# gicheonkang/gst-visdial

Hardware: AMD Instinct MI355X
Metric: dialog-rounds/sec (enc_dec_a train step) (higher is better)
Workload: dtype bf16; 1 GPU; enc_dec_a train step (fwd+loss+bwd+allreduce+AdamW, dropout on), 16 rows/GPU, seq_len 256, 37x2048 region features, answer len 25 [BASELINE configs[1] per-GPU shape]; global_batch=16, rows_per_gpu=16, seq_len=256, parallelism=dp1, hip_graph=True, optimizer_update=in the weight-gradient launch's epilogue + remainder pass, payload_written_by_wgrad_launch=False, capture_quiesce=no-process-group, full=False

## Files before the change

### gst_visdial_amd/_lib.py

```python
import ctypes as C
import os

_HERE = os.path.dirname(os.path.abspath(__file__))
LIB_PATH = os.path.join(_HERE, "lib", "libgstvd_hip.so")
ABI_VERSION = 9

F32, BF16 = 0, 1
EPI_BIAS, EPI_ADD, EPI_GELU, EPI_DGELU, EPI_DROPOUT = 1, 2, 4, 8, 16
EPI_COLSUM, EPI_COLSUM_ACC = 32, 64
EPI_ADAMW = 128
LN_RESID, LN_EMBED, LN_IMAGE = 0, 1, 2

_vp, _i64, _i32, _f32, _u32 = C.c_void_p, C.c_int64, C.c_int32, C.c_float, C.c_uint32


class GemmDesc(C.Structure):
    _fields_ = [("A", _vp), ("B", _vp), ("C", _vp), ("bias", _vp), ("addend", _vp), ("aux", _vp),
                ("M", _i64), ("N", _i64), ("K", _i64),
                ("lda", _i64), ("ldb", _i64), ("ldc", _i64), ("ldadd", _i64), ("ldaux", _i64),
                ("batch", _i64), ("sA", _i64), ("sB", _i64), ("sC", _i64), ("sAdd", _i64), ("sAux", _i64),
                ("dtype_in", _i32), ("dtype_out", _i32), ("a_kmajor", _i32), ("b_kmajor", _i32), ("epilogue", _i32),
                ("alpha", _f32), ("dropout_p", _f32), ("site", _u32), ("rng", _vp)]


# ... 76 lines not shown
    _fields_ = [("partial", _vp), ("out", _vp * 3), ("nblk", _i64), ("stride", _i64), ("H", _i64),
                ("nvec", _i32), ("accumulate", _i32 * 3), ("blk0", _i32)]


class SlabEntry(C.Structure):
    _fields_ = [("x", _vp), ("scratch", _vp), ("ldx", _i64), ("M", _i64), ("N", _i64), ("blk0", _i32), ("pad_", _i32)]


SIGNATURES = {
    "gstvd_abi_version": (_i32, []),
    "gstvd_build_arch": (C.c_char_p, []),
    "gstvd_gemm": (_i32, [C.POINTER(GemmDesc), _vp]),
    "gstvd_gemm_splitk_ws_bytes": (_i64, [_i64, _i64, _i32]),
    "gstvd_gemm_splitk": (_i32, [_vp, _i32, _vp, _i64, _vp]),
    "gstvd_gemm_group_tile": (_i32, []),
    "gstvd_gemm_group_caps": (_i32, []),
    "gstvd_gemv_ln": (_i32, [C.POINTER(GemmDesc), _vp, _vp, _f32, _vp, _i64, _vp]),
    "gstvd_gemm_kernel_name": (_i32, [C.POINTER(GemmDesc), _i32, C.c_char_p, _i32]),
    "gstvd_gemm_grouped_kernel_name": (_i32, [_i32, _i32, _i32, _i32, C.c_char_p, _i32]),
    "gstvd_gemm_grouped": (_i32, [_vp, _vp, _i64, _i64, _i32, _i32, _i32, _i32, _vp, _i64, _vp]),
    "gstvd_ln_fwd": (_i32, [C.POINTER(LnDesc), _vp]),
    "gstvd_ln_bwd_blocks": (_i64, [_i64]),
    "gstvd_ln_bwd_blocks_for": (_i64, [_i64, _i64, _i32]),
    "gstvd_ln_bwd": (_i32, [C.POINTER(LnBwdDesc), _vp]),
    "gstvd_gemm_ln_fwd": (_i32, [C.POINTER(GemmDesc), C.POINTER(LnDesc), _vp]),
    "gstvd_gemm_ln_bwd": (_i32, [C.POINTER(GemmDesc), C.POINTER(LnBwdDesc), _vp]),
    "gstvd_gemm_ln_rows_per_block": (_i64, []),
    "gstvd_colsum_partials": (_i32, [_vp, _i64, _i64, _i64, _vp, _vp, _vp, _i32, _vp]),
    "gstvd_colsum_batched": (_i32, [_vp, _i64, _i64, _vp]),
    "gstvd_colsum_slabs_batched": (_i32, [_vp, _i64, _i64, _i32, _vp]),
    "gstvd_colsum_slabs": (_i32, [_vp, _i64, _i64, _i64, _i32, _vp, _i64, _vp]),
    "gstvd_colsum": (_i32, [_vp, _i64, _i64, _i64, _i32, _vp, _vp, _i64, _i32, _vp]),
    "gstvd_locgrad": (_i32, [_vp, _i64, _vp, _i64, _i64, _i32, _vp, _i32, _vp]),
    "gstvd_attn_fwd": (_i32, [C.POINTER(AttnDesc), _vp]),
    "gstvd_attn_bwd": (_i32, [C.POINTER(AttnDesc), _vp]),
    "gstvd_ln_kernel_name": (_i32, [_vp, _i32, C.c_char_p, _i32]),
    "gstvd_attn_kernel_name": (_i32, [C.POINTER(AttnDesc), _i32, C.c_char_p, _i32]),
    "gstvd_ce_fwd": (_i32, [_vp, _i64, _vp, _i64, _i64, _i64, _i32, _vp, _vp, _vp, _vp]),
    "gstvd_ce_bwd": (_i32, [_vp, _i64, _vp, _vp, _vp, _vp, _i32, _i64, _i64, _i64, _i32, _vp, _i64, _vp]),
    "gstvd_ce_bwd_rows": (_i32, [_vp, _i64, _vp, _vp, _vp, _i64, _i64, _i64, _i32, _vp, _i64, _vp]),
    "gstvd_fgsm_step": (_i32, [_vp, _vp, _f32, _vp, _i64, _vp]),
    "gstvd_answer_scores": (_i32, [_vp, _i64, _vp, _vp, _i64, _i64, _i32, _vp, _vp]),
    "gstvd_sample_topk": (_i32, [C.POINTER(SampleDesc), _vp]),
    "gstvd_vl_split": (_i32, [_vp, _i64, _i64, _i64, _i64, _i32, _vp, _vp, _f32, _u32, _u32, _vp, _vp]),
    "gstvd_cast": (_i32, [_vp, _i32, _vp, _i32, _i64, _vp]),
    "gstvd_cast_ranges": (_i32, [_vp, _vp, _vp, _vp, _i64, _i64, _vp]),
    "gstvd_scale": (_i32, [_vp, _vp, _i64, _vp]),
    "gstvd_rng_advance": (_i32, [_vp, _vp]),
    "gstvd_dropout_mask": (_i32, [_vp, _i64, _f32, _u32, _vp, _vp]),
    "gstvd_adamw": (_i32, [_vp, _vp, _vp, _vp, _vp, _i64, _vp, _vp, _i64, _f32, _f32, _f32, _vp, _f32, _i64, _vp]),
    "gstvd_adamw_bf16grad": (_i32, [_vp, _vp, _i64, _vp, _vp, _vp, _i64, _vp, _vp, _i64, _f32, _f32, _f32, _vp, _f32, _i64, _vp]),
    "gstvd_adamw_blocks": (_i32, [_vp, _vp, _vp, _vp, _vp, _i64, _vp, _vp, _i64, _f32, _f32, _f32, _vp, _f32, _i64, _vp, _i64, _vp, _vp]),
    "gstvd_gemm_grouped_adamw": (_i32, [_vp, _vp, _i64, _i64, C.POINTER(AdamFuse), _vp, _i64, _vp]),
    "gstvd_gemm_grouped_adamw_kernel_name": (_i32, [C.c_char_p, _i32]),
    "gstvd_nsp_head": (_i32, [C.POINTER(NspHeadDesc), _vp]),
    "gstvd_rows_gather": (_i32, [_vp, _i64, _i64, _vp, _i64, _i64, _i32, _vp, _i64, _vp]),
    "gstvd_rows_scatter": (_i32, [_vp, _i64, _vp, _i64, _i64, _i32, _vp, _i64, _i64, _i32, _vp]),
    "gstvd_rows_mul": (_i32, [_vp, _i64, _vp, _i64, _i64, _i64, _i32, _vp]),
    "gstvd_kl_fwd": (_i32, [_vp, _i64, _vp, _i64, _vp, _vp, _i64, _i64, _i32, _vp, _vp, _vp, _vp]),
    "gstvd_kl_bwd": (_i32, [_vp, _i64, _vp, _i64, _vp, _vp, _vp, _vp, _vp, _i32, _i64, _i64, _i32, _vp, _i64, _vp]),
    "gstvd_nsp_train_fwd": (_i32, [C.POINTER(NspTrainDesc), _vp]),
    "gstvd_nsp_train_bwd": (_i32, [C.POINTER(NspTrainDesc), _vp]),
    "gstvd_beam_step": (_i32, [C.POINTER(BeamStepDesc), _vp]),
    "gstvd_beam_reorder": (_i32, [C.POINTER(BeamReorderDesc), _vp]),
}

_STATUS = {-1: "GSTVD_E_DTYPE", -2: "GSTVD_E_SHAPE", -3: "GSTVD_E_ALIGN", -4: "GSTVD_E_NULL", -5: "GSTVD_E_UNSUPPORTED"}


class GstvdError(RuntimeError):
    pass


_lib = None


def load():
    global _lib
    if _lib is not None:
        return _lib
    if not os.path.exists(LIB_PATH):
        raise GstvdError(
            "gst_visdial_amd: HIP library %s not found; build it first (make -C gst_visdial_amd/csrc). "
            "There is no CPU fallback for the product path." % LIB_PATH)
    import torch
    lib = C.CDLL(LIB_PATH)
    for name, (res, args) in SIGNATURES.items():
        fn = getattr(lib, name)
        fn.restype = res
        fn.argtypes = args
    if lib.gstvd_abi_version() != ABI_VERSION:
        raise GstvdError("libgstvd_hip.so ABI %d != expected %d; rebuild" % (lib.gstvd_abi_version(), ABI_VERSION))
    _lib = lib
    return lib


N_CALLS = [0]


def check(name, rc):
    N_CALLS[0] += 1
    if rc != 0:
        what = _STATUS.get(rc, "hipError_t %d" % rc if rc > 0 else "status %d" % rc)
        raise GstvdError("%s failed: %s" % (name, what))
```

### gst_visdial_amd/csrc/gemm_dma256.hip

```cpp
#include "gemm_common.h"

static __device__ __attribute__((aligned(256))) char g_zero_page256[256];
static constexpr int g_strip_w = 8;
constexpr int NS256 = 3;

DEVFN int opaque_lane(int lane) { asm volatile("" : "+v"(lane)); return lane; }
DEVFN int rm32_off(int row, int slot) { return row * 64 + ((slot ^ (((row >> 3) & 1) << 1)) << 4); }
template <int BX> DEVFN int km32_off(int krow, int col) {
  constexpr int NB = BX / 16;
  const int f = (krow & 3) | (((krow >> 3) & 1) << 2);
  return krow * (BX * 2) + ((((col >> 4) ^ f) & (NB - 1)) << 5) + ((col & 15) << 1);
}

template <int BX, bool KM> DEVFN bf16x8 frag32(const char* img, int xb, int lane) {
  const int g = lane >> 4, li = lane & 15;
  if (!KM) {
    return *(const bf16x8*)(img + rm32_off(xb + li, g));
  } else {
    const int kr = 8 * g + (li >> 2), col = xb + 4 * (lane & 3);
    s16x4 lo = lds_tr16(img + km32_off<BX>(kr, col));
    s16x4 hi = lds_tr16(img + km32_off<BX>(kr + 4, col));
    typedef __attribute__((ext_vector_type(8))) short s16x8;
    s16x8 v = {lo[0], lo[1], lo[2], lo[3], hi[0], hi[1], hi[2], hi[3]};
    return __builtin_bit_cast(bf16x8, v);
// ... 106 lines not shown
  }
#pragma unroll
  for (int i = 0; i < MI; ++i)
#pragma unroll
    for (int j = 0; j < NI; ++j)
      gemm_epilogue_tile<bf16, OT>(p, dk, acc[i][j], z, m0 + wm * WTM + i * 16 + li, n0 + wn * WTN + j * 16 + 4 * g);
}

#ifndef ADAMW_PARK_DEPTH
#define ADAMW_PARK_DEPTH 5
#endif
template <int NI, int ROWS, int D>
DEVFN void adamw_rows_pass(const gstvd_adamw_fuse_t& af, float alpha, float lr, float wd, float bc, const float* park, int64_t flat0,
                           int rows_left, int cols_left, unsigned ldc, int lane) {
  static_assert(NI == 4, "16 lanes x 4 columns = the wave tile's 64 columns");
  constexpr int S = epi_row_floats<NI>(), RPI = 4, R = ROWS / RPI;
  if (rows_left <= 0 || cols_left <= 0) return;
  const int rl = lane >> 4, c4 = (lane & 15) * 4;
  const bool n_ok = c4 < cols_left;
  float* Pt = af.param + flat0; float* Mt = af.m + flat0; float* Vt = af.v + flat0;
  bf16* St = (bf16*)af.shadow_bf16 + flat0;
  float* Gt = const_cast<float*>(af.grad_base) + flat0;
  const unsigned cofs = n_ok ? (unsigned)c4 : 0u;
  const int last = rows_left - 1;
  f32x4 bm[D + 1], bv[D + 1], bp[D + 1];
  auto fetch = [&](int rr, int b) {
    const int row = rr * RPI + rl;
    const unsigned o = (unsigned)(row < last ? row : last) * ldc + cofs;
    bm[b] = __builtin_nontemporal_load((const f32x4*)(Mt + o)); bv[b] = __builtin_nontemporal_load((const f32x4*)(Vt + o));
    bp[b] = __builtin_nontemporal_load((const f32x4*)(Pt + o));
  };
#pragma unroll
  for (int k = 0; k < D; ++k) fetch(k, k);
#pragma unroll
  for (int rr = 0; rr < R; ++rr) {
    if (rr + D < R) fetch(rr + D, (rr + D) % (D + 1));
    const int b = rr % (D + 1);
    const int row = rr * RPI + rl;
    f32x4 g4 = *(const f32x4*)(park + row * S + c4);
    g4 = g4 * alpha;
    f32x4 p4 = bp[b], m4 = bm[b], v4 = bv[b];
    adamw_update4(p4, m4, v4, g4, af.grad_scale, lr, wd, bc, af.beta1, af.beta2, af.eps);
    if (row < rows_left && n_ok) {
      const unsigned o = (unsigned)row * ldc + (unsigned)c4;
      if (af.write_grad) st4(Gt + o, g4);
      __builtin_nontemporal_store(m4, (f32x4*)(Mt + o));
      __builtin_nontemporal_store(v4, (f32x4*)(Vt + o));
      __builtin_nontemporal_store(p4, (f32x4*)(Pt + o));
      if (af.shadow_bf16) st4(St + o, p4);
    }
  }
}

template <typename OT, bool AKM, bool BKM, int NIU = 4, bool CS = false, bool ADAM = false>
DEVFN void pc_tile256(const GemmP& p, int64_t z, int wg, int ntn, int nwg, char* smem, const gstvd_adamw_fuse_t af = gstvd_adamw_fuse_t{}) {
  constexpr int BM = 256, BN = 256, WN = 4, NS = NS256, NTP = 256;
  constexpr int WTM = 128, WTN = NIU * 16, MI = 8, NI = NIU, BNU = WN * WTN;
  constexpr int A_BYTES = BM * 64, B_BYTES = BN * 64, STAGE = A_BYTES + B_BYTES;
  constexpr int NPA = A_BYTES / (NTP * 16), NPB = B_BYTES / (NTP * 16), LPS = NPA + NPB;
  static_assert((NS - 2) * LPS <= 63, "vmcnt immediate out of range");

  const int tid = threadIdx.x, lane = tid & 63;
  const int wave = __builtin_amdgcn_readfirstlane(tid >> 6);
  const bool producer = wave >= 8;
  const int ntm = nwg / ntn;
  const int SWD = g_strip_w;
  const int strip = wg / (SWD * ntm), sw = (ntn - strip * SWD) < SWD ? (ntn - strip * SWD) : SWD;
  const int within = wg - strip * SWD * ntm;
  const int64_t m0 = (int64_t)(within / sw) * BM, n0 = (int64_t)(strip * SWD + within % sw) * BNU;
  const int64_t nkt = (p.K + 31) / 32;

  if (producer) {
    const int ptid = tid - 512, pw = wave - 8;
    Dma32<BM, AKM, NPA, NTP> ua;
    Dma32<BN, BKM, NPB, NTP> ub;
    ua.init(p.A + z * p.sA * 2, p.lda, m0, p.M, ptid);
    ub.init(p.B + z * p.sB * 2, p.ldb, n0, (n0 + BNU < p.N) ? n0 + BNU : p.N, ptid);
#pragma unroll
    for (int s = 0; s < NS - 1; ++s) {
      ua.issue(s, p.K, smem + s * STAGE, pw);
      ub.issue(s, p.K, smem + s * STAGE + A_BYTES, pw);
    }
    int fill = NS - 1, slot = 0;
    const bool do_cs = CS && AKM && (p.epi & GSTVD_EPI_COLSUM) && n0 == 0 && p.bias != nullptr;
    const int rg = lane >> 3, cg = pw * 8 + (lane & 7);
    float cs[8] = {0.f, 0.f, 0.f, 0.f, 0.f, 0.f, 0.f, 0.f};
    for (int64_t t = 0; t < nkt; ++t) {
      asm volatile("s_waitcnt vmcnt(%0)" ::"n"((NS - 2) * LPS) : "memory");
      __builtin_amdgcn_s_barrier();
      asm volatile("" ::: "memory");
      ua.issue(t + NS - 1, p.K, smem + fill * STAGE, pw);
      ub.issue(t + NS - 1, p.K, smem + fill * STAGE + A_BYTES, pw);
      if (CS && do_cs) {
        const char* cA = smem + slot * STAGE;
#pragma unroll
        for (int r = 0; r < 4; ++r) {
          const bf16x8 v = *(const bf16x8*)(cA + km32_off<BM>(rg * 4 + r, cg * 8));
#pragma unroll
          for (int e = 0; e < 8; ++e) cs[e] += (float)v[e];
        }
        asm volatile("s_waitcnt lgkmcnt(0)" ::: "memory");
      }
      fill = (fill + 1 == NS) ? 0 : fill + 1;
      slot = (slot + 1 == NS) ? 0 : slot + 1;
    }
    asm volatile("s_waitcnt vmcnt(0)" ::: "memory");
    __builtin_amdgcn_s_barrier();
    if (CS && do_cs) {
#pragma unroll
      for (int e = 0; e < 8; ++e) {
        float v = cs[e];
        v += __shfl_xor(v, 8, 64);
        v += __shfl_xor(v, 16, 64);
        v += __shfl_xor(v, 32, 64);
        cs[e] = v;
      }
      if (rg == 0) {
// ... 213 lines not shown
          const bf16x8 fa = *(const bf16x8*)(cA + rm64_off(wm * WTM + i * 16 + li, h * 4 + g));
#pragma unroll
          for (int j = 0; j < NI; ++j) acc[i][j] = mfma_bf16_k32(fb[j], fa, acc[i][j]);
        }
      }
    }
    sa = (sa + 1 == 3) ? 0 : sa + 1;
    sb ^= 1;
  }
  }
  __builtin_amdgcn_s_barrier();
  const int lane_e = sizeof(OT) == 4 ? opaque_lane(lane) : lane;
  const int g = lane_e >> 4, li = lane_e & 15;
  const DropKey dk = make_drop((p.epi & GSTVD_EPI_DROPOUT) ? p.p : 0.f, p.site, p.rng);
  if constexpr (sizeof(OT) == 2) {
    if (epilogue_rows_ok(p)) {
      gemm_epilogue_rows<MI, NI, 4, (NIU >= 4)>(p, dk, acc, z, m0 + wm * WTM, n0 + wn * WTN, smem + wave * epi_wave_bytes<NI, 4>(), lane_e);
      return;
    }
  }
#pragma unroll
  for (int i = 0; i < MI; ++i) {
    const int li_i = opaque_lane(li), g_i = opaque_lane(g);
#pragma unroll
    for (int j = 0; j < NI; ++j)
      gemm_epilogue_tile<bf16, OT>(p, dk, acc[i][j], z, m0 + wm * WTM + i * 16 + li_i, n0 + wn * WTN + j * 16 + 4 * g_i);
  }
}

DEVFN int xcd_remap256(int bid, int nwg) {
  const int xcd = bid & 7, q = nwg >> 3, r = nwg & 7;
  return (xcd < r ? xcd * (q + 1) : r * (q + 1) + (xcd - r) * q) + (bid >> 3);
}

template <typename OT, bool AKM, bool BKM, int NIU = 4>
__global__ __launch_bounds__(512) void gemm_dma256_kernel(GemmP p, int ntn, int nwg) {
  extern __shared__ __attribute__((aligned(16))) char smem[];
  dma_tile256<OT, AKM, BKM, NIU>(p, blockIdx.y, xcd_remap256(blockIdx.x, nwg), ntn, nwg, smem);
}

template <typename OT, bool AKM, bool BKM, int NIU = 4>
__global__ __launch_bounds__(768) void gemm_pc256_kernel(GemmP p, int ntn, int nwg) {
  extern __shared__ __attribute__((aligned(16))) char smem[];
  pc_tile256<OT, AKM, BKM, NIU>(p, blockIdx.y, xcd_remap256(blockIdx.x, nwg), ntn, nwg, smem);
}

template <typename OT, int NIU>
__global__ __launch_bounds__(768) void gemm_pc256_nt64_kernel(GemmP p, int ntn, int nwg) {
  extern __shared__ __attribute__((aligned(16))) char smem[];
  pc_tile256_nt64<OT, NIU>(p, blockIdx.y, xcd_remap256(blockIdx.x, nwg), ntn, nwg, smem);
}

constexpr int GROUP_TILE_MASK = 0x1fffff;
DEVFN int grouped_tile_id(const int* bmap, int total, int chs) {
  const int bid = blockIdx.x;
  if (bmap) return bmap[bid];
  const int full = total - total % (8 << chs);
  return bid < full ? (((bid >> 3) >> chs) * 8 + (bid & 7)) * (1 << chs) + ((bid >> 3) & ((1 << chs) - 1)) : bid;
}

DEVFN GemmP grouped_problem(const gstvd_gemm_t* tab, const int* tile_off, int nprob, int gid, int& tile, int& ntn, int& nwg) {
  int lo = 0, hi = nprob - 1;
  while (lo < hi) { const int mid = (lo + hi + 1) >> 1; if (tile_off[mid] <= gid) lo = mid; else hi = mid - 1; }
  const gstvd_gemm_t& g = tab[lo];
  GemmP p;
  p.A = (const char*)g.A; p.B = (const char*)g.B; p.C = (char*)g.C;
  p.bias = g.bias; p.addend = (const char*)g.addend; p.aux = (char*)g.aux;
  p.M = g.M; p.N = g.N; p.K = g.K;
  p.lda = g.lda; p.ldb = g.ldb; p.ldc = g.ldc; p.ldadd = g.ldadd; p.ldaux = g.ldaux;
  p.sA = p.sB = p.sC = p.sAdd = p.sAux = 0;
  p.epi = g.epilogue; p.alpha = g.alpha; p.p = g.dropout_p; p.site = g.site; p.rng = g.rng;
  ntn = (int)((g.N + 255) / 256);
  nwg = (int)((g.M + 255) / 256) * ntn;
  tile = gid - tile_off[lo];
  return p;
}

template <typename OT, bool AKM, bool BKM>
__global__ __launch_bounds__(768) void gemm_pc256_grouped_kernel(const gstvd_gemm_t* tab, const int* tile_off, int nprob, int total, int chs,
                                                                 const int* bmap) {
  extern __shared__ __attribute__((aligned(16))) char smem[];
  const int entry = grouped_tile_id(bmap, total, chs);
  if (entry < 0 || (entry & GROUP_TILE_MASK) >= total) return;
  int tile, ntn, nwg;
  const GemmP p = grouped_problem(tab, tile_off, nprob, entry & GROUP_TILE_MASK, tile, ntn, nwg);
  pc_tile256<OT, AKM, BKM, 4, true>(p, 0, tile, ntn, nwg, smem);
}

__global__ __launch_bounds__(768) void gemm_pc256_grouped_adamw_kernel(const gstvd_gemm_t* tab, const int* tile_off, int nprob, int total, int chs,
                                                                       const int* bmap, gstvd_adamw_fuse_t af) {
  extern __shared__ __attribute__((aligned(16))) char smem[];
  const int entry = grouped_tile_id(bmap, total, chs);
  if (entry < 0 || (entry & GROUP_TILE_MASK) >= total) return;
  int tile, ntn, nwg;
  const GemmP p = grouped_problem(tab, tile_off, nprob, entry & GROUP_TILE_MASK, tile, ntn, nwg);
  pc_tile256<float, true, true, 4, true, true>(p, 0, tile, ntn, nwg, smem, af);
}

constexpr int RING256 = NS256 * (256 + 256) * 64;
constexpr int PARK256 = 8 * epi_wave_bytes<4, 4>();
constexpr int LDS256 = RING256 > PARK256 ? RING256 : PARK256;
constexpr int64_t PC256_MAX_TILES = 512;
constexpr int64_t GEMM256_MIN_TILES = 120;
constexpr int GROUP_CHUNK_LOG2 = 3;

template <typename OT, bool AKM, bool BKM>
static int launch256(const GemmP& p, int64_t batch, int niu, hipStream_t s) {
  const int bnu = niu == 3 ? 192 : 256;
  const int ntm = (int)((p.M + 255) / 256), ntn = (int)((p.N + bnu - 1) / bnu);
  const dim3 grid((unsigned)(ntm * ntn), (unsigned)batch);
  if ((int64_t)ntm * ntn * batch > PC256_MAX_TILES) {
    auto k4 = gemm_dma256_kernel<OT, AKM, BKM, 4>;
    auto k3 = gemm_dma256_kernel<OT, AKM, BKM, 3>;
    static int attr_rc = ensure_lds(k4, LDS256) | ensure_lds(k3, LDS256);
    if (attr_rc) return attr_rc;
    GSTVD_LAUNCH(bnu == 192 ? k3 : k4, grid, dim3(512), LDS256, s, p, ntn, ntm * ntn);
    GSTVD_LAUNCH_CHECK();
    return 0;
  }
  if constexpr (!AKM && !BKM) {
    if (p.K % 64 == 0 && p.K >= 128) {
      auto n4 = gemm_pc256_nt64_kernel<OT, 4>;
      auto n3 = gemm_pc256_nt64_kernel<OT, 3>;
      constexpr int L4 = 3 * 256 * 128 + 2 * 256 * 128, L3 = 3 * 256 * 128 + 2 * 192 * 128;
      constexpr int P4 = 8 * epi_wave_bytes<4, 4>(), P3 = 8 * epi_wave_bytes<3, 4>();
      constexpr int lds4 = L4 > P4 ? L4 : P4, lds3 = L3 > P3 ? L3 : P3;
      static_assert(lds4 <= 160 * 1024 && lds3 <= 160 * 1024, "LDS budget");
      static int nt_rc = ensure_lds(n4, lds4) | ensure_lds(n3, lds3);
      if (nt_rc) return nt_rc;
      GSTVD_LAUNCH(bnu == 192 ? n3 : n4, grid, dim3(768), bnu == 192 ? lds3 : lds4, s, p, ntn, ntm * ntn);
      GSTVD_LAUNCH_CHECK();
      return 0;
    }
  }
  auto c4 = gemm_pc256_kernel<OT, AKM, BKM, 4>;
  auto c3 = gemm_pc256_kernel<OT, AKM, BKM, 3>;
  static int pc_rc = ensure_lds(c4, LDS256) | ensure_lds(c3, LDS256);
  if (pc_rc) return pc_rc;
  GSTVD_LAUNCH(bnu == 192 ? c3 : c4, grid, dim3(768), LDS256, s, p, ntn, ntm * ntn);
  GSTVD_LAUNCH_CHECK();
  return 0;
}

template <typename OT>
static int launch256_layout(const GemmP& p, int64_t batch, int akm, int bkm, int niu, hipStream_t s) {
  if (!akm && !bkm) return launch256<OT, false, false>(p, batch, niu, s);
  if (!akm && bkm) return launch256<OT, false, true>(p, batch, niu, s);
  if (akm && bkm) return launch256<OT, true, true>(p, batch, niu, s);
  return GSTVD_E_UNSUPPORTED;
}

static int pick_niu(const GemmP& p, int64_t batch) {
  const double nkt = (double)((p.K + 31) / 32), ntm = (double)((p.M + 255) / 256);
  const double t4 = ntm * (double)((p.N + 255) / 256) * batch, t3 = ntm * (double)((p.N + 191) / 192) * batch;
  const double r4 = (double)(int64_t)((t4 + 255) / 256), r3 = (double)(int64_t)((t3 + 255) / 256);
  return r3 * (14.0 + 0.84 * nkt) < r4 * (14.0 + 0.95 * nkt) ? 3 : 4;
}

int gemm_dma256_dispatch(const GemmP& p, int64_t batch, int akm, int bkm, int out_f32, hipStream_t s) {
  const int64_t tiles = ((p.M + 255) / 256) * ((p.N + 255) / 256) * batch;
  if (p.M < 256 || p.N < 256 || tiles < GEMM256_MIN_TILES) return GSTVD_E_UNSUPPORTED;
  const int niu = pick_niu(p, batch);
  return out_f32 ? launch256_layout<float>(p, batch, akm, bkm, niu, s) : launch256_layout<bf16>(p, batch, akm, bkm, niu, s);
}

template <typename OT, bool AKM, bool BKM>
static int grouped256(const gstvd_gemm_t* tab, const int* off, int nprob, int total, const int* bmap, int nblocks, hipStream_t s) {
  auto kp = gemm_pc256_grouped_kernel<OT, AKM, BKM>;
  static int pc_rc = ensure_lds(kp, LDS256);
  if (pc_rc) return pc_rc;
  GSTVD_LAUNCH(kp, dim3((unsigned)(bmap ? nblocks : total)), dim3(768), LDS256, s, tab, off, nprob, total, GROUP_CHUNK_LOG2, bmap);
  GSTVD_LAUNCH_CHECK();
  return 0;
}

extern "C" int gstvd_gemm_group_tile(void) { return 256; }

extern "C" int32_t gstvd_gemm_group_caps(void) { return 1; }

extern "C" int gstvd_gemm_grouped_kernel_name(int32_t dtype_in, int32_t dtype_out, int32_t a_kmajor, int32_t b_kmajor, char* buf,
                                              int32_t buf_len) {
  if (!buf || buf_len <= 1) return GSTVD_E_NULL;
  const void* fn = nullptr;
  static gstvd_gemm_t dummy_tab;
  static int32_t dummy_off;
  gstvd_plan_capture = &fn;
  const int rc = gstvd_gemm_grouped(&dummy_tab, &dummy_off, 1, 1, dtype_in, dtype_out, a_kmajor, b_kmajor, nullptr, 0, nullptr);
  gstvd_plan_capture = nullptr;
  if (rc) return rc;
  return copy_kernel_name(fn, buf, buf_len);
}

extern "C" int gstvd_gemm_grouped_adamw_kernel_name(char* buf, int32_t buf_len) {
  if (!buf || buf_len <= 1) return GSTVD_E_NULL;
  return copy_kernel_name((const void*)gemm_pc256_grouped_adamw_kernel, buf, buf_len);
}

extern "C" int gstvd_gemm_grouped_adamw(const gstvd_gemm_t* table_dev, const int32_t* tile_off_dev, int64_t nprob, int64_t total_tiles,
                                        const gstvd_adamw_fuse_t* f, const int32_t* block_map_dev, int64_t nblocks, gstvd_stream_t stream) {
  if (!table_dev || !tile_off_dev || !f) return GSTVD_E_NULL;
  if (!f->grad_base || !f->param || !f->m || !f->v || !f->step) return GSTVD_E_NULL;
  if (nprob <= 0 || total_tiles <= 0) return GSTVD_E_SHAPE;
  if (block_map_dev && (nblocks < total_tiles || total_tiles > GROUP_TILE_MASK)) return GSTVD_E_SHAPE;
  if (((uintptr_t)f->grad_base | (uintptr_t)f->param | (uintptr_t)f->m | (uintptr_t)f->v | (uintptr_t)f->shadow_bf16) & 15) return GSTVD_E_ALIGN;
  auto kp = gemm_pc256_grouped_adamw_kernel;
  static int rc = ensure_lds(kp, LDS256);
  if (rc) return rc;
  GSTVD_LAUNCH(kp, dim3((unsigned)(block_map_dev ? nblocks : total_tiles)), dim3(768), LDS256, (hipStream_t)stream, table_dev, tile_off_dev,
               (int)nprob, (int)total_tiles, GROUP_CHUNK_LOG2, block_map_dev, *f);
  GSTVD_LAUNCH_CHECK();
  return 0;
}

extern "C" int gstvd_gemm_grouped(const gstvd_gemm_t* table_dev, const int32_t* tile_off_dev, int64_t nprob, int64_t total_tiles,
                                  int32_t dtype_in, int32_t dtype_out, int32_t a_kmajor, int32_t b_kmajor,
                                  const int32_t* block_map_dev, int64_t nblocks, gstvd_stream_t stream) {
  if (!table_dev || !tile_off_dev) return GSTVD_E_NULL;
  if (nprob <= 0 || total_tiles <= 0) return GSTVD_E_SHAPE;
  if (block_map_dev && (nblocks < total_tiles || total_tiles > GROUP_TILE_MASK)) return GSTVD_E_SHAPE;
  if (dtype_in != GSTVD_BF16) return GSTVD_E_UNSUPPORTED;
  hipStream_t s = (hipStream_t)stream;
  const int n = (int)nprob, t = (int)total_tiles, nb = (int)nblocks;
  const int* bm = block_map_dev;
  if (dtype_out == GSTVD_F32) {
    if (a_kmajor && b_kmajor) return grouped256<float, true, true>(table_dev, tile_off_dev, n, t, bm, nb, s);
    if (!a_kmajor && b_kmajor) return grouped256<float, false, true>(table_dev, tile_off_dev, n, t, bm, nb, s);
    if (!a_kmajor && !b_kmajor) return grouped256<float, false, false>(table_dev, tile_off_dev, n, t, bm, nb, s);
  } else if (dtype_out == GSTVD_BF16) {
    if (a_kmajor && b_kmajor) return grouped256<bf16, true, true>(table_dev, tile_off_dev, n, t, bm, nb, s);
    if (!a_kmajor && b_kmajor) return grouped256<bf16, false, true>(table_dev, tile_off_dev, n, t, bm, nb, s);
    if (!a_kmajor && !b_kmajor) return grouped256<bf16, false, false>(table_dev, tile_off_dev, n, t, bm, nb, s);
  }
  return GSTVD_E_UNSUPPORTED;
}
```

### gst_visdial_amd/ops.py

```python
import ctypes as C

import torch

from . import _lib as L
from ._lib import F32, BF16, EPI_BIAS, EPI_ADD, EPI_GELU, EPI_DGELU, EPI_DROPOUT, LN_RESID, LN_EMBED, LN_IMAGE

_DT = {torch.float32: F32, torch.bfloat16: BF16}


def dt(t):
    return _DT[t.dtype]


def _p(t):
    if t is None:
        return None
    if not t.is_cuda:
        raise L.GstvdError("gst_visdial_amd ops need GPU tensors (got %s); there is no CPU path" % t.device)
    return t.data_ptr()


_RAW_STREAM = getattr(torch._C, "_cuda_getCurrentRawStream", None)
_DEV_INDEX = None

# ... 261 lines not shown

    def add(self, A, B, C_out, M, N, K, accumulate, colsum_out=None, colsum_acc=False):
        di, do = dt(A), dt(C_out)
        if self.items and (di, do) != (self.dtype_in, self.dtype_out):
            self.flush()
        self.dtype_in, self.dtype_out = di, do
        self.keep.append((A, B, C_out, colsum_out))
        cs = (_p(colsum_out), int(bool(colsum_acc))) if colsum_out is not None else (0, 0)
        self.items.append((_p(A), _p(B), _p(C_out), M, N, K, A.stride(-2), B.stride(-2), C_out.stride(-2), int(bool(accumulate))) + cs)

    def reset(self):
        self.items, self.keep = [], []

    def pending_into(self, C_out):
        ptr = _p(C_out)
        return any(it[2] == ptr for it in self.items)

    @staticmethod
    def _overlapping(items):
        spans = sorted((it[2], it[2] + 4 * ((it[3] - 1) * it[8] + it[4]), i) for i, it in enumerate(items))
        bad, reach, owner = set(), -1, -1
        for lo, hi, i in spans:
            if lo < reach:
                bad.add(i); bad.add(owner)
            if hi > reach:
                reach, owner = hi, i
        return bad

    def flush_direct_bf16(self, G, Gb):
        if not self.items or self.dtype_in != BF16 or self.dtype_out != F32 or not (self.a_km and self.b_km):
            self.flush()
            return ()
        base, nG = G.data_ptr(), G.numel()
        shared = self._overlapping(self.items)
        direct, rest, keep_d, keep_r, ranges = [], [], [], [], []
        for i, (it, kp) in enumerate(zip(self.items, self.keep)):
            (a, b, c, M, N, K, lda, ldb, ldc, acc) = it[:10]
            off = (c - base) // 4
            if acc or i in shared or ldc != N or c < base or off + M * N > nG or (c - base) % 4 or off % 8:
                rest.append(it); keep_r.append(kp)
            else:
                direct.append(it[:2] + (Gb.data_ptr() + 2 * off,) + it[3:]); keep_d.append(kp)
                ranges.append((off, M * N))
        self.items, self.keep = rest, keep_r
        self.flush()
        if direct:
            self.items, self.keep, self.dtype_out = direct, keep_d, BF16
            try:
                self.flush()
            finally:
                self.dtype_out = F32
        return tuple(sorted(ranges))

    def flush(self, fuse=None):
        if not self.items:
            return ()
        keep, self.keep = self.keep, []
        fused = ()
        if fuse is not None and self.dtype_in == BF16 and self.dtype_out == F32 and self.a_km and self.b_km:
            items, fl = [], []
            shared = self._overlapping(self.items)
            for i, it in enumerate(self.items):
                (a, b, c, M, N, K, lda, ldb, ldc, acc, cs_ptr, cs_acc) = it[:12]
                hp_addr, offs = (0, ()) if (acc or i in shared) else fuse.cover(c, M, N, ldc)
                fl.extend(offs)
                items.append(it[:12] + (hp_addr,))
            if fl:
                self.items, fused = items, tuple(fl)
            else:
                fuse = None
        else:
            fuse = None
        if self.dtype_in != BF16:
            lib = L.load()
            for (a, b, c, M, N, K, lda, ldb, ldc, acc, cs_ptr, cs_acc) in [it[:12] for it in self.items]:
                if cs_ptr:
                    raise L.GstvdError("column sums ride on the grouped bf16 launch only")
                d = L.GemmDesc()
                d.A, d.B, d.C, d.M, d.N, d.K, d.lda, d.ldb, d.ldc, d.batch = a, b, c, M, N, K, lda, ldb, ldc, 1
                d.dtype_in, d.dtype_out, d.a_kmajor, d.b_kmajor, d.alpha = self.dtype_in, self.dtype_out, int(self.a_km), int(self.b_km), 1.0
                if acc:
                    d.addend, d.ldadd, d.epilogue = c, ldc, EPI_ADD
                L.check("gstvd_gemm", lib.gstvd_gemm(C.byref(d), _stream()))
            self.items = []
            return ()
        key = tuple(self.items)
        hit = self.cache.get(key)
        if hit is None:
            arr = (L.GemmDesc * len(key))()
            offs, tiles, flops, nbytes = [], 0, 0.0, 0.0
            esz_in, esz_out = (2 if self.dtype_in == BF16 else 4), (2 if self.dtype_out == BF16 else 4)
            T = int(L.load().gstvd_gemm_group_tile())
            for d, it in zip(arr, key):
                (a, b, c, M, N, K, lda, ldb, ldc, acc, cs_ptr, cs_acc) = it[:12]
                d.A, d.B, d.C, d.M, d.N, d.K, d.lda, d.ldb, d.ldc, d.batch = a, b, c, M, N, K, lda, ldb, ldc, 1
                d.dtype_in, d.dtype_out, d.a_kmajor, d.b_kmajor, d.alpha = self.dtype_in, self.dtype_out, int(self.a_km), int(self.b_km), 1.0
                if acc:
                    d.addend, d.ldadd, d.epilogue = c, ldc, EPI_ADD
                elif len(it) > 12 and it[12]:
                    d.addend, d.epilogue = it[12], L.EPI_ADAMW
                if cs_ptr:
                    d.bias = cs_ptr
                    d.epilogue |= L.EPI_COLSUM | (L.EPI_COLSUM_ACC if cs_acc else 0)
                offs.append(tiles)
                tiles += ((M + T - 1) // T) * ((N + T - 1) // T)
                flops += 2.0 * M * N * K
                if len(it) > 12 and it[12]:
                    nbytes += esz_in * (M * K + K * N) + M * N * 26.0
                else:
                    nbytes += esz_in * (M * K + K * N) + esz_out * M * N * (2 if acc else 1)
            tab = torch.frombuffer(bytearray(bytes(arr)), dtype=torch.uint8).to(self.device)
            off = torch.tensor(offs, dtype=torch.int32).to(self.device)
            bmap = None
            if GROUP_ORDER and tiles >= GROUP_ORDER_MIN_TILES:
                mode = 3 if fuse is not None else 1
                bm_host = xcd_block_map([(it[3], it[4], it[5]) for it in key], T, fuse is not None, mode)
                if sorted(t for t in bm_host if t >= 0) != list(range(tiles)) or any(t < -1 for t in bm_host):
                    raise L.GstvdError("internal: block map is not a placement of the launch's %d tiles" % tiles)
                bmap = torch.tensor(bm_host, dtype=torch.int32).to(self.device)
            hit = (tab, off, len(key), tiles, flops, nbytes, bmap)
            if len(self.cache) > 64:
                self.cache.clear()
            self.cache[key] = hit
        tab, off, n, tiles, flops, nbytes, bmap = hit
        bm_ptr, bm_n = (bmap.data_ptr(), bmap.numel()) if bmap is not None else (None, 0)
        lib = L.load()
        e0 = _prof_begin()
        if fuse is not None:
            L.check("gstvd_gemm_grouped_adamw", lib.gstvd_gemm_grouped_adamw(tab.data_ptr(), off.data_ptr(), n, tiles, C.byref(fuse.desc()),
                                                                             bm_ptr, bm_n, _stream()))
            if e0 is not None:
                name = _KNAME.get("grouped_adamw")
                if name is None:
                    buf = C.create_string_buffer(512)
                    L.check("gstvd_gemm_grouped_adamw_kernel_name", lib.gstvd_gemm_grouped_adamw_kernel_name(buf, 512))
                    name = _KNAME["grouped_adamw"] = buf.value.decode()
                _prof_end(e0, "gemm:" + name, flops, nbytes, (n, tiles))
            self.items = []
            return fused
        L.check("gstvd_gemm_grouped", lib.gstvd_gemm_grouped(tab.data_ptr(), off.data_ptr(), n, tiles, self.dtype_in, self.dtype_out,
                                                             int(self.a_km), int(self.b_km), bm_ptr, bm_n, _stream()))
        if e0 is not None:
            key = ("grouped", self.dtype_in, self.dtype_out, self.a_km, self.b_km)
            name = _KNAME.get(key)
            if name is None:
                buf = C.create_string_buffer(512)
                L.check("gstvd_gemm_grouped_kernel_name", lib.gstvd_gemm_grouped_kernel_name(self.dtype_in, self.dtype_out, int(self.a_km),
                                                                                           int(self.b_km), buf, 512))
                name = _KNAME[key] = buf.value.decode()
            _prof_end(e0, "gemm:" + name, flops, nbytes, (n, tiles))
        self.items = []
        return ()


def _ln_desc(mode, dtype, M, H, gamma, beta, mean, rstd, eps, x=None, res=None, y=None, p_pre=0.0, p_post=0.0,
             site_pre=0, site_post=0, rng=None, ids=None, segs=None, T=0, type_vocab=2, word=None, pos=None, tt=None,
             tt_ext=None, loc=None, w_loc=None, b_loc=None, pos_offset=0):
    d = L.LnDesc()
    d.mode, d.dtype, d.M, d.H = mode, dtype, M, H
    d.x, d.ldx = _p(x), (x.stride(-2) if x is not None else 0)
    d.res, d.ldres = _p(res), (res.stride(-2) if res is not None else 0)
    d.gamma, d.beta, d.eps = _p(gamma), _p(beta), eps
    d.y, d.ldy = _p(y), (y.stride(-2) if y is not None else 0)
    d.mean, d.rstd = _p(mean), _p(rstd)
    d.p_pre, d.p_post, d.site_pre, d.site_post = p_pre, p_post, site_pre, site_post
    d.rng = rng.ptr() if (rng is not None and (p_pre > 0 or p_post > 0)) else None
    d.ids, d.segs, d.T, d.type_vocab = _p(ids), _p(segs), T, type_vocab
    d.word, d.pos, d.tt, d.tt_ext = _p(word), _p(pos), _p(tt), _p(tt_ext)
    d.loc, d.w_loc, d.b_loc = _p(loc), _p(w_loc), _p(b_loc)
    d.pos_offset = pos_offset
    return d


def ln_fwd(**kw):
    lib = L.load()
    d = _ln_desc(**kw)
    e0 = _prof_begin()
    L.check("gstvd_ln_fwd", lib.gstvd_ln_fwd(C.byref(d), _stream()))
    _prof_end(e0, "ln_fwd", 0.0, 3.0 * d.M * d.H * (2 if d.dtype == BF16 else 4), (d.M, d.H, d.mode))


def ln_bwd_blocks(M, H=None, mode=None):
    if H is None:
# ... 635 lines not shown
```

### include/gstvd_hip.h

```cpp
#ifndef GSTVD_HIP_H
#define GSTVD_HIP_H

#include <stdint.h>

#ifdef __cplusplus
extern "C" {
#endif

typedef void* gstvd_stream_t;

enum { GSTVD_F32 = 0, GSTVD_BF16 = 1 };
enum {
  GSTVD_E_DTYPE = -1, GSTVD_E_SHAPE = -2, GSTVD_E_ALIGN = -3, GSTVD_E_NULL = -4, GSTVD_E_UNSUPPORTED = -5
};

int gstvd_abi_version(void);
const char* gstvd_build_arch(void);

enum { GSTVD_EPI_BIAS = 1, GSTVD_EPI_ADD = 2, GSTVD_EPI_GELU = 4, GSTVD_EPI_DGELU = 8, GSTVD_EPI_DROPOUT = 16,
       GSTVD_EPI_COLSUM = 32, GSTVD_EPI_COLSUM_ACC = 64,
       GSTVD_EPI_ADAMW = 128 };

typedef struct {
  const void* A; const void* B; void* C;
// ... 91 lines not shown
int gstvd_attn_bwd(const gstvd_attn_t* a, gstvd_stream_t s);
int gstvd_attn_kernel_name(const gstvd_attn_t* a, int32_t bwd, char* buf, int32_t buf_len);

int gstvd_ce_fwd(const void* logits, int64_t ldl, const int64_t* labels, int64_t M, int64_t V,
                 int64_t ignore_index, int32_t dtype, float* row_loss, float* lse, float* stats,
                 gstvd_stream_t s);
int gstvd_ce_bwd(const void* logits, int64_t ldl, const int64_t* labels, const float* lse,
                 const float* stats, const float* gscale, int32_t mean, int64_t M, int64_t V,
                 int64_t ignore_index, int32_t dtype, void* dlogits, int64_t ldd, gstvd_stream_t s);
int gstvd_ce_bwd_rows(const void* logits, int64_t ldl, const int64_t* labels, const float* lse, const float* g, int64_t M,
                      int64_t V, int64_t ignore_index, int32_t dtype, void* dlogits, int64_t ldd, gstvd_stream_t s);
int gstvd_fgsm_step(const float* x, const float* g, float eps, float* out, int64_t n, gstvd_stream_t s);
int gstvd_answer_scores(const void* logits, int64_t ldl, const float* lse, const int64_t* dec_ids,
                        int64_t rows, int64_t U, int32_t dtype, float* scores, gstvd_stream_t s);

typedef struct {
  const void* logits; int64_t ld; int32_t dtype; int32_t B; int32_t V; int32_t top_k; float temperature;
  const float* u; int64_t* out; int64_t out_stride; const uint8_t* banned; int64_t banned_ld;
  const int64_t* hist; int64_t hist_ld; int32_t hist_T; int32_t ngram;
  const int64_t* ids_tm; int64_t ids_stride; int32_t cur_len; int32_t n_special; int32_t special[8];
  float top_p; int32_t reserved_;
} gstvd_sample_t;
int gstvd_sample_topk(const gstvd_sample_t* a, gstvd_stream_t s);

int gstvd_vl_split(const void* d_enc, int64_t B, int64_t R, int64_t T, int64_t H, int32_t dtype, void* d_v, void* d_t,
                   float p, uint32_t site_v, uint32_t site_t, const uint64_t* rng, gstvd_stream_t s);

int gstvd_cast(const void* src, int32_t src_dtype, void* dst, int32_t dst_dtype, int64_t n, gstvd_stream_t s);
int gstvd_cast_ranges(const float* src, void* dst_bf16, const int64_t* ranges_dev, const int32_t* blk0_dev, int64_t nranges,
                      int64_t total_blocks, gstvd_stream_t s);
int gstvd_scale(float* x, const float* factor, int64_t n, gstvd_stream_t s);
int gstvd_rng_advance(uint64_t* rng, gstvd_stream_t s);
int gstvd_dropout_mask(float* out, int64_t n, float p, uint32_t site, const uint64_t* rng, gstvd_stream_t s);

int gstvd_adamw(float* param, const float* grad, float* m, float* v, void* shadow_bf16, int64_t n,
                const int64_t* seg_end, const float* hp, int64_t nseg, float beta1, float beta2, float eps,
                const float* step , float grad_scale, int64_t begin, gstvd_stream_t s);
int gstvd_adamw_bf16grad(float* param, const void* grad_bf16, int64_t grad_origin, float* m, float* v, void* shadow_bf16,
                         int64_t n, const int64_t* seg_end, const float* hp, int64_t nseg, float beta1, float beta2, float eps,
                         const float* step, float grad_scale, int64_t begin, gstvd_stream_t s);

int gstvd_adamw_blocks(float* param, const float* grad, float* m, float* v, void* shadow_bf16, int64_t n,
                       const int64_t* seg_end, const float* hp, int64_t nseg, float beta1, float beta2, float eps,
                       const float* step, float grad_scale, int64_t begin, const int32_t* block_list_dev, int64_t nblocks,
                       const uint8_t* seg_skip_dev, gstvd_stream_t s);

typedef struct {
  const float* grad_base; float* param; float* m; float* v; void* shadow_bf16;
  const float* step; float beta1, beta2, eps, grad_scale;
  int32_t write_grad;
} gstvd_adamw_fuse_t;
int gstvd_gemm_grouped_adamw(const gstvd_gemm_t* table_dev, const int32_t* tile_off_dev, int64_t nprob, int64_t total_tiles,
                             const gstvd_adamw_fuse_t* f, const int32_t* block_map_dev, int64_t nblocks, gstvd_stream_t s);
int gstvd_gemm_grouped_adamw_kernel_name(char* buf, int32_t buf_len);

int gstvd_gemv_ln(const gstvd_gemm_t* g, const float* gamma, const float* beta, float eps, void* y_out, int64_t ldy, gstvd_stream_t s);
int32_t gstvd_gemm_group_caps(void);
int gstvd_gemm_kernel_name(const gstvd_gemm_t* g, int32_t splits, char* buf, int32_t buf_len);
int gstvd_gemm_grouped_kernel_name(int32_t dtype_in, int32_t dtype_out, int32_t a_kmajor, int32_t b_kmajor, char* buf, int32_t buf_len);

typedef struct {
  const void* xt; int64_t ldt; int64_t t_rows;
  const void* xv; int64_t ldv; int64_t v_rows;
  const void* wt; int64_t ldwt; const void* wv; int64_t ldwv;
  const float* bt; const float* bv; const float* wn; int64_t ldwn; const float* bn;
  float* z; int64_t ldz; float* prob0;
  int32_t B, H, Hv, Hb, dtype, fusion;
  char* kernel_name; int32_t kernel_name_len; int32_t reserved_;
} gstvd_nsp_head_t;
int gstvd_nsp_head(const gstvd_nsp_head_t* a, gstvd_stream_t s);

int gstvd_rows_gather(const void* src, int64_t lds, int64_t M, const int64_t* idx, int64_t n, int64_t H, int32_t dtype,
                      void* dst, int64_t ldd, gstvd_stream_t s);
int gstvd_rows_scatter(const void* src, int64_t lds, const int64_t* idx, int64_t n, int64_t H, int32_t dtype, void* dst,
                       int64_t ldd, int64_t M, int32_t accumulate, gstvd_stream_t s);

int gstvd_rows_mul(void* x, int64_t ldx, const void* a, int64_t lda, int64_t M, int64_t N, int32_t dtype, gstvd_stream_t s);

int gstvd_kl_fwd(const void* scores, int64_t lds, const float* target, int64_t ldt, const int64_t* target_row,
                 const int64_t* labels, int64_t rows, int64_t C, int32_t dtype, float* row_loss, float* lse, float* stats,
                 gstvd_stream_t s);
int gstvd_kl_bwd(const void* scores, int64_t lds, const float* target, int64_t ldt, const int64_t* target_row,
                 const int64_t* labels, const float* lse, const float* stats, const float* gscale, int32_t mean,
                 int64_t rows, int64_t C, int32_t dtype, void* dscores, int64_t ldd, gstvd_stream_t s);

typedef struct {
  const void* xt; int64_t ldt; int64_t t_rows;
  const void* xv; int64_t ldv; int64_t v_rows;
  const void* wt; int64_t ldwt; const void* wv; int64_t ldwv;
  const float* bt; const float* bv; const float* wn; int64_t ldwn; const float* bn;
  const float* labels; int64_t ldl;
  float* z; int64_t ldz;
  float* pt; float* pv; uint8_t* keep; float* row_loss; float* stats;
  const float* gscale; float* dwn; int64_t lddwn; float* dbn; void* dpt; void* dpv; int64_t lddp;
  const uint64_t* rng; float p; uint32_t site;
  int32_t B, H, Hv, Hb, dtype, fusion, acc_w, acc_b;
  char* kernel_name; int32_t kernel_name_len; int32_t reserved_;
} gstvd_nsp_train_t;
int gstvd_nsp_train_fwd(const gstvd_nsp_train_t* a, gstvd_stream_t s);
int gstvd_nsp_train_bwd(const gstvd_nsp_train_t* a, gstvd_stream_t s);

typedef struct {
  const void* logits; int64_t ld; int32_t dtype; int32_t B; int32_t K; int32_t V;
  const float* score_in; const int32_t* done_in;
  float* score_out; int32_t* done_out; int32_t* parent;
  int64_t* ids_tm; int64_t ids_stride; int32_t positions; int32_t pos;
// ... 18 lines not shown
```

Measured before the change: 1359 dialog-rounds/sec.

## Make grouped wgrad+AdamW kernel persistent with role-specialized grid-stride tile walk

Adds a grid-size parameter to the fused weight-gradient/AdamW grouped GEMM so workgroups can loop over multiple tile entries with a barrier between tiles. Producer and consumer waves are specialized at compile time, and the tile table and block map are read through the constant address space. The aim is to cut the cost of launching many short-lived workgroups and to make scalar loads cheaper. With the default grid of one workgroup per entry, behaviour mostly stays the same; a bounded grid would add serialization and LDS reuse hazards across tiles.

```diff
diff --git a/gst_visdial_amd/_lib.py b/gst_visdial_amd/_lib.py
--- a/gst_visdial_amd/_lib.py
+++ b/gst_visdial_amd/_lib.py
@@ -152,6 +152,7 @@
     "gstvd_adamw_bf16grad": (_i32, [_vp, _vp, _i64, _vp, _vp, _vp, _i64, _vp, _vp, _i64, _f32, _f32, _f32, _vp, _f32, _i64, _vp]),
     "gstvd_adamw_blocks": (_i32, [_vp, _vp, _vp, _vp, _vp, _i64, _vp, _vp, _i64, _f32, _f32, _f32, _vp, _f32, _i64, _vp, _i64, _vp, _vp]),
     "gstvd_gemm_grouped_adamw": (_i32, [_vp, _vp, _i64, _i64, C.POINTER(AdamFuse), _vp, _i64, _vp]),
+    "gstvd_gemm_grouped_adamw_grid": (_i32, [_vp, _vp, _i64, _i64, C.POINTER(AdamFuse), _vp, _i64, _i64, _vp]),
     "gstvd_gemm_grouped_adamw_kernel_name": (_i32, [C.c_char_p, _i32]),
     "gstvd_nsp_head": (_i32, [C.POINTER(NspHeadDesc), _vp]),
     "gstvd_rows_gather": (_i32, [_vp, _i64, _i64, _vp, _i64, _i64, _i32, _vp, _i64, _vp]),
diff --git a/gst_visdial_amd/csrc/gemm_dma256.hip b/gst_visdial_amd/csrc/gemm_dma256.hip
--- a/gst_visdial_amd/csrc/gemm_dma256.hip
+++ b/gst_visdial_amd/csrc/gemm_dma256.hip
@@ -182,7 +182,7 @@
   }
 }
 
-template <typename OT, bool AKM, bool BKM, int NIU = 4, bool CS = false, bool ADAM = false>
+template <typename OT, bool AKM, bool BKM, int NIU = 4, bool CS = false, bool ADAM = false, int ROLE = 0>
 DEVFN void pc_tile256(const GemmP& p, int64_t z, int wg, int ntn, int nwg, char* smem, const gstvd_adamw_fuse_t af = gstvd_adamw_fuse_t{}) {
   constexpr int BM = 256, BN = 256, WN = 4, NS = NS256, NTP = 256;
   constexpr int WTM = 128, WTN = NIU * 16, MI = 8, NI = NIU, BNU = WN * WTN;
@@ -190,9 +190,9 @@
   constexpr int NPA = A_BYTES / (NTP * 16), NPB = B_BYTES / (NTP * 16), LPS = NPA + NPB;
   static_assert((NS - 2) * LPS <= 63, "vmcnt immediate out of range");
 
-  const int tid = threadIdx.x, lane = tid & 63;
+  const int tid = ADAM ? opaque_lane(threadIdx.x) : (int)threadIdx.x, lane = tid & 63;
   const int wave = __builtin_amdgcn_readfirstlane(tid >> 6);
-  const bool producer = wave >= 8;
+  const bool producer = ROLE == 1 || (ROLE == 0 && wave >= 8);
   const int ntm = nwg / ntn;
   const int SWD = g_strip_w;
   const int strip = wg / (SWD * ntm), sw = (ntn - strip * SWD) < SWD ? (ntn - strip * SWD) : SWD;
@@ -512,17 +512,19 @@
 }
 
 constexpr int GROUP_TILE_MASK = 0x1fffff;
-DEVFN int grouped_tile_id(const int* bmap, int total, int chs) {
-  const int bid = blockIdx.x;
+#define CONST_AS __attribute__((address_space(4)))
+template <typename IP>
+DEVFN int grouped_tile_id(IP bmap, int total, int chs, int bid) {
   if (bmap) return bmap[bid];
-  const int full = total - total % (8 << chs);
+  const int full = total & ~((8 << chs) - 1);
   return bid < full ? (((bid >> 3) >> chs) * 8 + (bid & 7)) * (1 << chs) + ((bid >> 3) & ((1 << chs) - 1)) : bid;
 }
 
-DEVFN GemmP grouped_problem(const gstvd_gemm_t* tab, const int* tile_off, int nprob, int gid, int& tile, int& ntn, int& nwg) {
+template <typename TP, typename IP>
+DEVFN GemmP grouped_problem(TP tab, IP tile_off, int nprob, int gid, int& tile, int& ntn, int& nwg) {
   int lo = 0, hi = nprob - 1;
   while (lo < hi) { const int mid = (lo + hi + 1) >> 1; if (tile_off[mid] <= gid) lo = mid; else hi = mid - 1; }
-  const gstvd_gemm_t& g = tab[lo];
+  const auto& g = tab[lo];
   GemmP p;
   p.A = (const char*)g.A; p.B = (const char*)g.B; p.C = (char*)g.C;
   p.bias = g.bias; p.addend = (const char*)g.addend; p.aux = (char*)g.aux;
@@ -540,21 +542,39 @@
 __global__ __launch_bounds__(768) void gemm_pc256_grouped_kernel(const gstvd_gemm_t* tab, const int* tile_off, int nprob, int total, int chs,
                                                                  const int* bmap) {
   extern __shared__ __attribute__((aligned(16))) char smem[];
-  const int entry = grouped_tile_id(bmap, total, chs);
+  const int entry = grouped_tile_id(bmap, total, chs, blockIdx.x);
   if (entry < 0 || (entry & GROUP_TILE_MASK) >= total) return;
   int tile, ntn, nwg;
   const GemmP p = grouped_problem(tab, tile_off, nprob, entry & GROUP_TILE_MASK, tile, ntn, nwg);
   pc_tile256<OT, AKM, BKM, 4, true>(p, 0, tile, ntn, nwg, smem);
 }
 
+template <int ROLE>
+DEVFN void grouped_adamw_walk(const gstvd_gemm_t* tab_g, const int* tile_off_g, int nprob, int total, int chs, const int* bmap_g, int nblocks,
+                              const gstvd_adamw_fuse_t& af, char* smem) {
+  const CONST_AS gstvd_gemm_t* tab = (const CONST_AS gstvd_gemm_t*)tab_g;
+  const CONST_AS int* tile_off = (const CONST_AS int*)tile_off_g;
+  const CONST_AS int* bmap = (const CONST_AS int*)bmap_g;
+  const int first = blockIdx.x, stride = gridDim.x;
+  for (int b = first; b < nblocks; b += stride) {
+    if (b != first) {
+      asm volatile("s_waitcnt lgkmcnt(0)" ::: "memory");
+      __builtin_amdgcn_s_barrier();
+      asm volatile("" ::: "memory");
+    }
+    const int entry = grouped_tile_id(bmap, total, chs, b);
+    if (entry < 0 || (entry & GROUP_TILE_MASK) >= total) continue;
+    int tile, ntn, nwg;
+    const GemmP p = grouped_problem(tab, tile_off, nprob, entry & GROUP_TILE_MASK, tile, ntn, nwg);
+    pc_tile256<float, true, true, 4, true, true, ROLE>(p, 0, tile, ntn, nwg, smem, af);
+  }
+}
+
 __global__ __launch_bounds__(768) void gemm_pc256_grouped_adamw_kernel(const gstvd_gemm_t* tab, const int* tile_off, int nprob, int total, int chs,
-                                                                       const int* bmap, gstvd_adamw_fuse_t af) {
+                                                                       const int* bmap, int nblocks, gstvd_adamw_fuse_t af) {
   extern __shared__ __attribute__((aligned(16))) char smem[];
-  const int entry = grouped_tile_id(bmap, total, chs);
-  if (entry < 0 || (entry & GROUP_TILE_MASK) >= total) return;
-  int tile, ntn, nwg;
-  const GemmP p = grouped_problem(tab, tile_off, nprob, entry & GROUP_TILE_MASK, tile, ntn, nwg);
-  pc_tile256<float, true, true, 4, true, true>(p, 0, tile, ntn, nwg, smem, af);
+  if (__builtin_amdgcn_readfirstlane(threadIdx.x >> 6) >= 8) grouped_adamw_walk<1>(tab, tile_off, nprob, total, chs, bmap, nblocks, af, smem);
+  else grouped_adamw_walk<2>(tab, tile_off, nprob, total, chs, bmap, nblocks, af, smem);
 }
 
 constexpr int RING256 = NS256 * (256 + 256) * 64;
@@ -656,20 +676,30 @@
   return copy_kernel_name((const void*)gemm_pc256_grouped_adamw_kernel, buf, buf_len);
 }
 
-extern "C" int gstvd_gemm_grouped_adamw(const gstvd_gemm_t* table_dev, const int32_t* tile_off_dev, int64_t nprob, int64_t total_tiles,
-                                        const gstvd_adamw_fuse_t* f, const int32_t* block_map_dev, int64_t nblocks, gstvd_stream_t stream) {
+extern "C" int gstvd_gemm_grouped_adamw_grid(const gstvd_gemm_t* table_dev, const int32_t* tile_off_dev, int64_t nprob, int64_t total_tiles,
+                                             const gstvd_adamw_fuse_t* f, const int32_t* block_map_dev, int64_t nblocks, int64_t grid_wgs,
+                                             gstvd_stream_t stream) {
   if (!table_dev || !tile_off_dev || !f) return GSTVD_E_NULL;
   if (!f->grad_base || !f->param || !f->m || !f->v || !f->step) return GSTVD_E_NULL;
   if (nprob <= 0 || total_tiles <= 0) return GSTVD_E_SHAPE;
   if (block_map_dev && (nblocks < total_tiles || total_tiles > GROUP_TILE_MASK)) return GSTVD_E_SHAPE;
+  const int64_t nb = block_map_dev ? nblocks : total_tiles;
+  if (nb > INT32_MAX) return GSTVD_E_SHAPE;
+  if (grid_wgs != nb && (grid_wgs <= 0 || grid_wgs % 8 != 0 || grid_wgs > nb)) return GSTVD_E_SHAPE;
   if (((uintptr_t)f->grad_base | (uintptr_t)f->param | (uintptr_t)f->m | (uintptr_t)f->v | (uintptr_t)f->shadow_bf16) & 15) return GSTVD_E_ALIGN;
   auto kp = gemm_pc256_grouped_adamw_kernel;
   static int rc = ensure_lds(kp, LDS256);
   if (rc) return rc;
-  GSTVD_LAUNCH(kp, dim3((unsigned)(block_map_dev ? nblocks : total_tiles)), dim3(768), LDS256, (hipStream_t)stream, table_dev, tile_off_dev,
-               (int)nprob, (int)total_tiles, GROUP_CHUNK_LOG2, block_map_dev, *f);
+  GSTVD_LAUNCH(kp, dim3((unsigned)grid_wgs), dim3(768), LDS256, (hipStream_t)stream, table_dev, tile_off_dev,
+               (int)nprob, (int)total_tiles, GROUP_CHUNK_LOG2, block_map_dev, (int)nb, *f);
   GSTVD_LAUNCH_CHECK();
   return 0;
+}
+
+extern "C" int gstvd_gemm_grouped_adamw(const gstvd_gemm_t* table_dev, const int32_t* tile_off_dev, int64_t nprob, int64_t total_tiles,
+                                        const gstvd_adamw_fuse_t* f, const int32_t* block_map_dev, int64_t nblocks, gstvd_stream_t stream) {
+  return gstvd_gemm_grouped_adamw_grid(table_dev, tile_off_dev, nprob, total_tiles, f, block_map_dev, nblocks,
+                                       block_map_dev ? nblocks : total_tiles, stream);
 }
 
 extern "C" int gstvd_gemm_grouped(const gstvd_gemm_t* table_dev, const int32_t* tile_off_dev, int64_t nprob, int64_t total_tiles,
diff --git a/gst_visdial_amd/ops.py b/gst_visdial_amd/ops.py
--- a/gst_visdial_amd/ops.py
+++ b/gst_visdial_amd/ops.py
@@ -337,7 +337,13 @@
                 self.dtype_out = F32
         return tuple(sorted(ranges))
 
-    def flush(self, fuse=None):
+    @staticmethod
+    def bounded_grid(grid_wgs, entries):
+        if grid_wgs is None or grid_wgs >= entries or entries <= N_XCD:
+            return entries
+        return max(N_XCD, grid_wgs - grid_wgs % N_XCD)
+
+    def flush(self, fuse=None, grid_wgs=None):
         if not self.items:
             return ()
         keep, self.keep = self.keep, []
@@ -369,9 +375,11 @@
                 L.check("gstvd_gemm", lib.gstvd_gemm(C.byref(d), _stream()))
             self.items = []
             return ()
-        key = tuple(self.items)
+        items = tuple(self.items)
+        key = (items, grid_wgs if fuse is not None else None)
         hit = self.cache.get(key)
         if hit is None:
+            key_, key = key, items
             arr = (L.GemmDesc * len(key))()
             offs, tiles, flops, nbytes = [], 0, 0.0, 0.0
             esz_in, esz_out = (2 if self.dtype_in == BF16 else 4), (2 if self.dtype_out == BF16 else 4)
@@ -403,17 +411,18 @@
                 if sorted(t for t in bm_host if t >= 0) != list(range(tiles)) or any(t < -1 for t in bm_host):
                     raise L.GstvdError("internal: block map is not a placement of the launch's %d tiles" % tiles)
                 bmap = torch.tensor(bm_host, dtype=torch.int32).to(self.device)
-            hit = (tab, off, len(key), tiles, flops, nbytes, bmap)
+            grid = self.bounded_grid(grid_wgs if fuse is not None else None, len(bm_host) if bmap is not None else tiles)
+            hit = (tab, off, len(key), tiles, flops, nbytes, bmap, grid)
             if len(self.cache) > 64:
                 self.cache.clear()
-            self.cache[key] = hit
-        tab, off, n, tiles, flops, nbytes, bmap = hit
+            self.cache[key_] = hit
+        tab, off, n, tiles, flops, nbytes, bmap, grid = hit
         bm_ptr, bm_n = (bmap.data_ptr(), bmap.numel()) if bmap is not None else (None, 0)
         lib = L.load()
         e0 = _prof_begin()
         if fuse is not None:
-            L.check("gstvd_gemm_grouped_adamw", lib.gstvd_gemm_grouped_adamw(tab.data_ptr(), off.data_ptr(), n, tiles, C.byref(fuse.desc()),
-                                                                             bm_ptr, bm_n, _stream()))
+            L.check("gstvd_gemm_grouped_adamw_grid", lib.gstvd_gemm_grouped_adamw_grid(tab.data_ptr(), off.data_ptr(), n, tiles,
+                                                                                       C.byref(fuse.desc()), bm_ptr, bm_n, grid, _stream()))
             if e0 is not None:
                 name = _KNAME.get("grouped_adamw")
                 if name is None:
diff --git a/include/gstvd_hip.h b/include/gstvd_hip.h
--- a/include/gstvd_hip.h
+++ b/include/gstvd_hip.h
@@ -167,6 +167,9 @@
 } gstvd_adamw_fuse_t;
 int gstvd_gemm_grouped_adamw(const gstvd_gemm_t* table_dev, const int32_t* tile_off_dev, int64_t nprob, int64_t total_tiles,
                              const gstvd_adamw_fuse_t* f, const int32_t* block_map_dev, int64_t nblocks, gstvd_stream_t s);
+int gstvd_gemm_grouped_adamw_grid(const gstvd_gemm_t* table_dev, const int32_t* tile_off_dev, int64_t nprob, int64_t total_tiles,
+                                  const gstvd_adamw_fuse_t* f, const int32_t* block_map_dev, int64_t nblocks, int64_t grid_wgs,
+                                  gstvd_stream_t s);
 int gstvd_gemm_grouped_adamw_kernel_name(char* buf, int32_t buf_len);
 
 int gstvd_gemv_ln(const gstvd_gemm_t* g, const float* gamma, const float* beta, float eps, void* y_out, int64_t ldy, gstvd_stream_t s);
```

Result: no change. 1360 dialog-rounds/sec (median of 2 runs) (+0.1%).
